# maxsonate/video-diffusion-nnx

Measured on AMD Instinct MI355X. Metric: denoised frames/sec, 16fx64x64 1000-step DDPM, higher is better.
Workload: dtype bf16; 1 GPU; config_v2_2 (north-star shape): Unet3D dim=64 C=1, 16f x 64x64, DDPM T=1000 p_sample_loop (UNet forward + p_sample per step, hipGraph replay); value = n_gpus*B*F/(T*s_per_step); batch_per_gpu=64, parallelism=dp1 (independent samples, no collective), mfma_operands=bf16, storage=weights fp32 master, activations bf16, fp32 accumulate, process_group=none (single process)

## Files before the change

video_diffusion_nnx_amd/csrc/conv_igemm.hip:

```cpp
#include "vdx_common.h"
#include <type_traits>
#include "vdx_internal.h"
#include "vdx_glds.h"
#include "model.h"
#include <stdlib.h>
#include <string.h>

namespace vdx {

typedef unsigned u32x4 __attribute__((ext_vector_type(4)));
typedef unsigned u32x2 __attribute__((ext_vector_type(2)));
constexpr unsigned OOB = 0xFFFFFFF0u;

template <int MODE, int BC, int TN, int NW, int INF>
__global__ __launch_bounds__(64 * NW, (NW == 8 && TN == 2) ? 4 : 2) void conv_igemm_kernel(const ConvArgs P) {
    using M = Mma<MODE>;
    constexpr int KT = M::KT;
    constexpr int RS = ROW_STRIDE;
    constexpr int WAVES_C = BC / 64;
    constexpr int WAVES_P = NW / WAVES_C;
    constexpr int NT = 64 * NW;
    constexpr int TM = 4;
    constexpr int APIECES = KT / 4;
    constexpr int WREGS = BC * 8 / NT;
// ... 689 lines not shown
        }
        {
            const int oy0 = tyc * 16 + 2 * wave, ox = txc * 16 + lp;
#pragma unroll
            for (int tn = 0; tn < 2; ++tn) {
                const size_t gout = ((size_t)(fcur * P.H + oy0 + tn) * P.W + ox) * 64;
#pragma unroll
                for (int tm = 0; tm < 4; ++tm) {
                    float4 v = make_float4(acc[tm][tn][0] + bias4[tm].x, acc[tm][tn][1] + bias4[tm].y, acc[tm][tn][2] + bias4[tm].z, acc[tm][tn][3] + bias4[tm].w);
                    const float4 r4 = rpre[tm][tn]; v.x += r4.x; v.y += r4.y; v.z += r4.z; v.w += r4.w;
                    store4_f32_or_bf16(P.y, gout + tm * 16 + 4 * q, v, OUT16 ? 1 : 0);
                    ssum[tm][0] += v.x; ssum[tm][1] += v.y; ssum[tm][2] += v.z; ssum[tm][3] += v.w;
                    ssq[tm][0] += v.x * v.x; ssq[tm][1] += v.y * v.y; ssq[tm][2] += v.z * v.z; ssq[tm][3] += v.w * v.w;
                }
            }
        }
        wait_vm<8>();
        if (more && bn != bcur) { flush_stats(bcur); bcur = bn; }
        fcur = fn; tyc = tyn; txc = txn;
        __syncthreads();
    }
    flush_stats(bcur);
}

template <typename K>
static hipError_t launch_tiles16(K kfn, const ConvArgs& a, size_t lds, long slots, hipStream_t st) {
    const int total = a.NF * (a.H >> 4) * (a.W >> 4);
    const PersistentSplit s = persistent_split(total, slots);
    if (hipError_t e = lds_opt_in(kfn, lds); e != hipSuccess) return e;
    hipLaunchKernelGGL(kfn, dim3((unsigned)s.workers), dim3(512), lds, st, a, (int)s.per, total);
    return hipGetLastError();
}

static hipError_t launch_conv64d(const ConvArgs& a, hipStream_t st) {
    if (a.pro || !a.x0_bf16 || !a.res || a.res_bf16) return hipErrorInvalidValue;
    const size_t lds = 9 * 64 * 128 + 2 * (size_t)C64D_APL + 128 * 8;
    return launch_tiles16(a.y_bf16 ? conv64d_kernel<true, true> : conv64d_kernel<false, true>, a, lds, device_cus(), st);
}

template <bool OUT16>
__global__ __launch_bounds__(512) void conv64r_kernel(const ConvArgs P, const int tiles_per_block, const int total_tiles) {
    using M = Mma<MODE_BF16>;
    constexpr int NDMA = 41, NK = (NDMA + 7) / 8;
    extern __shared__ __attribute__((aligned(16))) char smem[];
    char* Al = smem;
    double* chs = reinterpret_cast<double*>(Al + 3 * C64D_APL);
    float* biasl = reinterpret_cast<float*>(chs + 128);

    const int tid = threadIdx.x, lane = tid & 63;
    const int wave_u = __builtin_amdgcn_readfirstlane(tid >> 6);
    const int wc = wave_u & 1, wp = wave_u >> 1;
    const int lp = lane & 15, q = lane >> 4;
    const int tiles_x = P.W >> 4, tiles_pf = tiles_x * (P.H >> 4);
    const int t0 = blockIdx.x * tiles_per_block, t1 = min(t0 + tiles_per_block, total_tiles);
    if (t0 >= t1) return;

    uint4 wf[9][2][2];
#pragma unroll
    for (int tap = 0; tap < 9; ++tap)
#pragma unroll
        for (int ch = 0; ch < 2; ++ch)
#pragma unroll
            for (int tm = 0; tm < 2; ++tm)
                wf[tap][ch][tm] = *reinterpret_cast<const uint4*>(reinterpret_cast<const char*>(P.wp) +
                    ((size_t)tap * P.wrows + P.wrow0 + wc * 32 + 8 * (lp >> 2) + 4 * tm + (lp & 3)) * 128 + ch * 64 + q * 16);
    if (tid < 128) chs[tid] = 0.0;
    if (tid < 64) biasl[tid] = P.bias ? P.bias[tid] : 0.f;

    const char* const zero_page = reinterpret_cast<const char*>(g_zero_page_c64d);
    const char* const xb = reinterpret_cast<const char*>(P.x0);
    const unsigned al_base = lds_addr(Al);
    auto decode = [&](int t, int& f, int& ty, int& tx) { f = t / tiles_pf; const int r = t - f * tiles_pf; ty = r / tiles_x; tx = r - ty * tiles_x; };
    auto dma = [&](int t, int buf) {
        int f, ty, tx; decode(t, f, ty, tx);
        int ln = lane;
        asm volatile("" : "+v"(ln));
        const unsigned dst = al_base + buf * C64D_APL + wave_u * 1024;
#pragma unroll
        for (int k = 0; k < NK; ++k) {
            if (wave_u + 8 * k >= NDMA) continue;
            const int hp = (wave_u + 8 * k) * 8 + (ln >> 3);
            const int hy = (hp * 3641) >> 16, hx = hp - hy * 18;
            const int gy = ty * 16 - 1 + hy, gx = tx * 16 - 1 + hx;
            const bool ok = hp < C64_HALO && gy >= 0 && gy < P.H && gx >= 0 && gx < P.W;
            const size_t off = (size_t)((f * P.H + gy) * P.W + gx) * 128 + (((ln & 7) ^ (hx & 7)) << 4);
            glds16(ok ? static_cast<const void*>(xb + off) : static_cast<const void*>(zero_page), dst + k * 8 * 1024);
        }
    };
    const __amdgpu_buffer_rsrc_t rsy = __builtin_amdgcn_make_buffer_rsrc(P.y, 0, (unsigned)P.NF * P.H * P.W * 64u * (OUT16 ? 2u : 4u), 0x00020000);
    f32x4 ssum[2], ssq[2];
#pragma unroll
    for (int i = 0; i < 2; ++i) { ssum[i] = f32x4{0.f, 0.f, 0.f, 0.f}; ssq[i] = f32x4{0.f, 0.f, 0.f, 0.f}; }
    auto flush_stats = [&](int b) {
        if (!P.out_stats) return;
#pragma unroll
        for (int tm = 0; tm < 2; ++tm)
#pragma unroll
            for (int e = 0; e < 4; ++e) {
                const float s1 = reduce16(ssum[tm][e]), s2 = reduce16(ssq[tm][e]);
                const int c = wc * 32 + 8 * q + 4 * tm + e;
                if (lp == 0) { unsafeAtomicAdd(&chs[c], (double)s1); unsafeAtomicAdd(&chs[64 + c], (double)s2); }
                ssum[tm][e] = 0.f; ssq[tm][e] = 0.f;
            }
        __syncthreads();
        const int cpg = 64 / P.out_groups;
        int tt = tid;
        asm volatile("" : "+v"(tt));
        if (tt < 2 * P.out_groups) {
            const int g = tt >> 1, which = tt & 1;
            double t = 0.0;
            for (int c = g * cpg; c < (g + 1) * cpg; ++c) t += chs[which * 64 + c];
            unsafeAtomicAdd(P.out_stats + (((size_t)b * GN_SLOTS + (blockIdx.x % GN_SLOTS)) * P.out_groups + g) * 2 + which, t);
        }
        __syncthreads();
        if (tid < 128) chs[tid] = 0.0;
        __syncthreads();
    };

    int bdx[3][2];
#pragma unroll
    for (int ch = 0; ch < 2; ++ch)
#pragma unroll
        for (int dx = 0; dx < 3; ++dx) { const int hx = lp + dx; bdx[dx][ch] = hx * 128 + 16 * ((q + 4 * ch) ^ (hx & 7)); }
    const int rowbase = (4 * wp) * 18 * 128;

    int fcur, tyc, txc;
    decode(t0, fcur, tyc, txc);
    int bcur = fcur / P.F;
    __syncthreads();
    dma(t0, 0);
    if (t0 + 1 < t1) { dma(t0 + 1, 1); wait_vm<5>(); } else wait_vm<0>();
    __syncthreads();
    int buf = 0;
    for (int t = t0; t < t1; ++t) {
        const bool more = t + 1 < t1, more2 = t + 2 < t1;
        int fn = fcur, tyn = tyc, txn = txc, bn = bcur;
        if (more) { decode(t + 1, fn, tyn, txn); bn = fn / P.F; }
        if (more2) dma(t + 2, buf >= 1 ? buf - 1 : 2);
        const char* At = Al + buf * C64D_APL + rowbase;
        const int oy0 = tyc * 16 + 4 * wp, ox = txc * 16 + lp;
        f32x4 acc[2][4];
        uint4 bf[2][3];
        auto frag_read = [&](uint4 (&d)[3], int hr, int ch) {
#pragma unroll
            for (int dx = 0; dx < 3; ++dx) d[dx] = *reinterpret_cast<const uint4*>(At + bdx[dx][ch] + hr * (18 * 128));
        };
        frag_read(bf[0], 0, 0);
#pragma unroll
        for (int hr = 0; hr < 6; ++hr) {
            if (hr < 4) { acc[0][hr] = f32x4{0.f, 0.f, 0.f, 0.f}; acc[1][hr] = f32x4{0.f, 0.f, 0.f, 0.f}; }
#pragma unroll
            for (int ch = 0; ch < 2; ++ch) {
                const int s_ = 2 * hr + ch;
                if (s_ + 1 < 12) frag_read(bf[(s_ + 1) & 1], (s_ + 1) >> 1, (s_ + 1) & 1);
                __builtin_amdgcn_sched_barrier(0);
#pragma unroll
                for (int dx = 0; dx < 3; ++dx)
#pragma unroll
                    for (int dy = 0; dy < 3; ++dy) {
                        const int tn = hr - dy;
                        if (tn < 0 || tn > 3) continue;
#pragma unroll
                        for (int tm = 0; tm < 2; ++tm) M::mma(acc[tm][tn], wf[dy * 3 + dx][ch][tm], bf[s_ & 1][dx]);
                    }
                __builtin_amdgcn_sched_barrier(0);
            }
            if (hr >= 2) {
                const int tn = hr - 2;
                float4 bias4[2];
#pragma unroll
                for (int tm = 0; tm < 2; ++tm) bias4[tm] = *reinterpret_cast<const float4*>(biasl + wc * 32 + 8 * q + 4 * tm);
                const unsigned gout = (unsigned)(((fcur * P.H + oy0 + tn) * P.W + ox) * 64 + wc * 32 + 8 * q);
                float4 v[2];
#pragma unroll
                for (int tm = 0; tm < 2; ++tm) {
                    v[tm] = make_float4(acc[tm][tn][0] + bias4[tm].x, acc[tm][tn][1] + bias4[tm].y, acc[tm][tn][2] + bias4[tm].z, acc[tm][tn][3] + bias4[tm].w);
                    ssum[tm][0] += v[tm].x; ssum[tm][1] += v[tm].y; ssum[tm][2] += v[tm].z; ssum[tm][3] += v[tm].w;
                    ssq[tm][0] += v[tm].x * v[tm].x; ssq[tm][1] += v[tm].y * v[tm].y; ssq[tm][2] += v[tm].z * v[tm].z; ssq[tm][3] += v[tm].w * v[tm].w;
                }
                if constexpr (OUT16)
                    __builtin_amdgcn_raw_buffer_store_b128(u32x4{pack_bf16x2(v[0].x, v[0].y), pack_bf16x2(v[0].z, v[0].w), pack_bf16x2(v[1].x, v[1].y), pack_bf16x2(v[1].z, v[1].w)}, rsy, gout * 2u, 0, 0);
                else {
#pragma unroll
                    for (int tm = 0; tm < 2; ++tm)
                        __builtin_amdgcn_raw_buffer_store_b128(u32x4{__float_as_uint(v[tm].x), __float_as_uint(v[tm].y), __float_as_uint(v[tm].z), __float_as_uint(v[tm].w)}, rsy, (gout + 4 * tm) * 4u, 0, 0);
                }
            }
        }
        constexpr int NST = OUT16 ? 4 : 8;
        if (more2) wait_vm<5 + NST>(); else wait_vm<NST>();
        if (more && bn != bcur) { flush_stats(bcur); bcur = bn; }
        fcur = fn; tyc = tyn; txc = txn;
        buf = buf == 2 ? 0 : buf + 1;
        __syncthreads();
    }
    flush_stats(bcur);
}

static hipError_t launch_conv64r(const ConvArgs& a, hipStream_t st) {
    if (a.pro || !a.x0_bf16 || a.res) return hipErrorInvalidValue;
    const size_t lds = 3 * (size_t)C64D_APL + 128 * 8 + 64 * 4;
    return launch_tiles16(a.y_bf16 ? conv64r_kernel<true> : conv64r_kernel<false>, a, lds, device_cus(), st);
}

#ifndef VDX_C64Q_VPM
#define VDX_C64Q_VPM 6
#endif
template <int CIN, bool PRO, bool OUT16, int COUT = 64>
__global__ __launch_bounds__(512) void conv64q_kernel(const ConvArgs P, const int tiles_per_block, const int total_tiles) {
    using M = Mma<MODE_BF16>;
    static_assert(CIN == 64 || (CIN == 128 && !PRO), "prologue form: 64 input channels");
    static_assert(COUT == 64 || (COUT == 32 && !PRO), "COUT");
    constexpr int NWC = COUT / 16, NWP = 8 / NWC, RW = 16 / NWP, NHR = RW + 2, NSTEP = 2 * NHR;
    constexpr int NPL = CIN / 64;
    constexpr int NDMA = 41, NK = (NDMA + 7) / 8;
    constexpr int NST = (OUT16 ? 1 : 2) * (RW / 2);
    extern __shared__ __attribute__((aligned(16))) char smem[];
    char* Al = smem;
    double* chs = reinterpret_cast<double*>(Al + 3 * C64D_APL);
    float* biasl = reinterpret_cast<float*>(chs + 128);
    float* coefA = biasl + 64;
    float* coefD = coefA + 64;
    float* gmean = coefD + 64;

    const int tid = threadIdx.x, lane = tid & 63;
    const int wave_u = __builtin_amdgcn_readfirstlane(tid >> 6);
    const int wc = wave_u % NWC, wp = wave_u / NWC;
    const int lp = lane & 15, q = lane >> 4;
    const int tiles_x = P.W >> 4, tiles_pf = tiles_x * (P.H >> 4);
    const int t0 = blockIdx.x * tiles_per_block, t1 = min(t0 + tiles_per_block, total_tiles);
    if (t0 >= t1) return;

    uint4 wf[9][CIN / 32];
#pragma unroll
    for (int tap = 0; tap < 9; ++tap)
#pragma unroll
        for (int c = 0; c < CIN / 32; ++c)
            wf[tap][c] = *reinterpret_cast<const uint4*>(reinterpret_cast<const char*>(P.wp) +
                ((size_t)tap * P.wrows + P.wrow0 + wc * 16 + lp) * (CIN * 2) + c * 64 + q * 16);
    if (tid < 128) chs[tid] = 0.0;
    if (tid < 64) biasl[tid] = (P.bias && tid < COUT) ? P.bias[tid] : 0.f;

    const char* const zero_page = reinterpret_cast<const char*>(g_zero_page_c64d);
    const char* const xb0 = reinterpret_cast<const char*>(P.x0);
    const char* const xb1 = (CIN == 128) ? (P.C1 ? reinterpret_cast<const char*>(P.x1) : xb0 + 128) : xb0;
    const int rowb = (CIN == 128 && !P.C1) ? 256 : 128;
    const bool split32 = CIN == 64 && P.C1 == 32;
    const char* const xs1 = split32 ? reinterpret_cast<const char*>(P.x1) : nullptr;
    const unsigned al_base = lds_addr(Al);
    auto decode = [&](int t, int& f, int& ty, int& tx) { f = t / tiles_pf; const int r = t - f * tiles_pf; ty = r / tiles_x; tx = r - ty * tiles_x; };
    auto dma = [&](int t, int plane, int buf) {
        int f, ty, tx; decode(t, f, ty, tx);
        int ln = lane;
        asm volatile("" : "+v"(ln));
        const char* const xb = plane ? xb1 : xb0;
        const unsigned dst = al_base + buf * C64D_APL + wave_u * 1024;
#pragma unroll
        for (int k = 0; k < NK; ++k) {
            if (wave_u + 8 * k >= NDMA) continue;
            const int hp = (wave_u + 8 * k) * 8 + (ln >> 3);
            const int hy = (hp * 3641) >> 16, hx = hp - hy * 18;
            const int gy = ty * 16 - 1 + hy, gx = tx * 16 - 1 + hx;
            const bool ok = hp < C64_HALO && gy >= 0 && gy < P.H && gx >= 0 && gx < P.W;
            const int cch = (ln & 7) ^ (hx & 7);
            const size_t pixi = (size_t)((f * P.H + gy) * P.W + gx);
            const char* src = split32 ? (cch < 4 ? xb0 : xs1) + pixi * 64 + ((cch & 3) << 4) : xb + pixi * rowb + (cch << 4);
            glds16(ok ? static_cast<const void*>(src) : static_cast<const void*>(zero_page), dst + k * 8 * 1024);
        }
    };
    const __amdgpu_buffer_rsrc_t rsy = __builtin_amdgcn_make_buffer_rsrc(P.y, 0, (unsigned)P.NF * P.H * P.W * (unsigned)COUT * (OUT16 ? 2u : 4u), 0x00020000);
    float ssum[8], ssq[8];
#pragma unroll
    for (int i = 0; i < 8; ++i) { ssum[i] = 0.f; ssq[i] = 0.f; }
    auto flush_stats = [&](int b) {
        if (!P.out_stats) return;
#pragma unroll
        for (int i = 0; i < 8; ++i) {
            const float s1 = reduce16(ssum[i]), s2 = reduce16(ssq[i]);
            const int c = wc * 16 + 8 * (q >> 1) + i;
            if (lp == 0) { unsafeAtomicAdd(&chs[c], (double)s1); unsafeAtomicAdd(&chs[64 + c], (double)s2); }
            ssum[i] = 0.f; ssq[i] = 0.f;
        }
        __syncthreads();
        const int cpg = COUT / P.out_groups;
        int tt = tid;
        asm volatile("" : "+v"(tt));
        if (tt < 2 * P.out_groups) {
            const int g = tt >> 1, which = tt & 1;
            double t = 0.0;
            for (int c = g * cpg; c < (g + 1) * cpg; ++c) t += chs[which * 64 + c];
            unsafeAtomicAdd(P.out_stats + (((size_t)b * GN_SLOTS + (blockIdx.x % GN_SLOTS)) * P.out_groups + g) * 2 + which, t);
        }
        __syncthreads();
        if (tid < 128) chs[tid] = 0.0;
        __syncthreads();
    };
    const int tch = tid & 7, trow = tid >> 3;
    float ca[PRO ? 8 : 1], cd[PRO ? 8 : 1];
    auto make_coef = [&](int b) {
        if constexpr (PRO) {
            gn_mean_rstd_wg(P.in_stats, b, P.groups, (double)P.F * P.H * P.W * (64 / P.groups), gmean, tid, 512);
            __syncthreads();
            int tt = tid;
            asm volatile("" : "+v"(tt));
            if (tt < 64) {
                const int g = tt / (64 / P.groups);
                const float m = gmean[2 * g], rsd = gmean[2 * g + 1];
                float sc = 1.f, sh = 0.f;
                if (P.ss) { sc = P.ss[(size_t)b * P.ss_stride + tt] + 1.f; sh = P.ss[(size_t)b * P.ss_stride + 64 + tt]; }
                coefA[tt] = rsd * P.gamma[tt] * sc;
                coefD[tt] = (P.beta[tt] - m * rsd * P.gamma[tt]) * sc + sh;
            }
            __syncthreads();
#pragma unroll
            for (int i = 0; i < 8; ++i) { ca[i] = coefA[8 * tch + i]; cd[i] = coefD[8 * tch + i]; }
        }
    };
    auto piece_off = [&](int k) __attribute__((always_inline)) -> int {
        const int hp = trow + 64 * k;
        const int hy = (hp * 3641) >> 16, hx = hp - hy * 18;
        return hp * 128 + ((tch ^ (hx & 7)) << 4);
    };
    auto piece_ok = [&](int k, int ty, int tx) __attribute__((always_inline)) -> bool {
        const int hp = trow + 64 * k;
// ... 101 lines not shown
                                if ((c & 1) == 0) {
                                    cur = pv; okc = pok;
                                    if (k + 1 < NPK - 1) { pv = *reinterpret_cast<const u32x4*>(An + piece_off(k + 1)); pok = piece_ok(k + 1, tyn, txn); }
                                    half_math(cur.x, cur.y, 0, okc, oh0, oh1);
                                } else {
                                    unsigned o2, o3;
                                    half_math(cur.z, cur.w, 4, okc, o2, o3);
                                    *reinterpret_cast<u32x4*>(An + piece_off(k)) = u32x4{oh0, oh1, o2, o3};
                                }
#pragma unroll
                                for (int i = 0; i < 9; ++i) { __builtin_amdgcn_sched_group_barrier(0x008, 1, 0); __builtin_amdgcn_sched_group_barrier(0x002, VDX_C64Q_VPM, 0); }
                            }
                        }
                        __builtin_amdgcn_sched_barrier(0);
                        if constexpr (XF) {
                            if (s_ == 14 && wave_u == 0 && trow + 64 * (NPK - 1) < C64D_AROWS) {
                                char* pp = An + piece_off(NPK - 1);
                                *reinterpret_cast<u32x4*>(pp) = piece_math(*reinterpret_cast<const u32x4*>(pp), piece_ok(NPK - 1, tyn, txn));
                            }
                        }
                    }
                    if (plane == NPL - 1 && hr >= 3 && (hr & 1)) {
                        const int ta = hr - 3;
                        float v[8];
#pragma unroll
                        for (int r = 0; r < 4; ++r) {
                            const auto sw = __builtin_amdgcn_permlane16_swap(__float_as_uint(acc[ta][r]), __float_as_uint(acc[ta + 1][r]), false, false);
                            v[r] = __uint_as_float(sw[0]); v[4 + r] = __uint_as_float(sw[1]);
                        }
                        const float4 b0 = *reinterpret_cast<const float4*>(biasl + wc * 16 + 8 * (q >> 1)), b1 = *reinterpret_cast<const float4*>(biasl + wc * 16 + 8 * (q >> 1) + 4);
                        v[0] += b0.x; v[1] += b0.y; v[2] += b0.z; v[3] += b0.w; v[4] += b1.x; v[5] += b1.y; v[6] += b1.z; v[7] += b1.w;
#pragma unroll
                        for (int i = 0; i < 8; ++i) { ssum[i] += v[i]; ssq[i] += v[i] * v[i]; }
                        const unsigned gout = (unsigned)(((fcur * P.H + oy0 + ta + (q & 1)) * P.W + ox) * COUT + wc * 16 + 8 * (q >> 1));
                        if constexpr (OUT16)
                            __builtin_amdgcn_raw_buffer_store_b128(u32x4{pack_bf16x2(v[0], v[1]), pack_bf16x2(v[2], v[3]), pack_bf16x2(v[4], v[5]), pack_bf16x2(v[6], v[7])}, rsy, gout * 2u, 0, 0);
                        else {
                            __builtin_amdgcn_raw_buffer_store_b128(u32x4{__float_as_uint(v[0]), __float_as_uint(v[1]), __float_as_uint(v[2]), __float_as_uint(v[3])}, rsy, gout * 4u, 0, 0);
                            __builtin_amdgcn_raw_buffer_store_b128(u32x4{__float_as_uint(v[4]), __float_as_uint(v[5]), __float_as_uint(v[6]), __float_as_uint(v[7])}, rsy, (gout + 4) * 4u, 0, 0);
                        }
                    }
                }
            };
            if (PRO && more) steps(std::true_type{}); else steps(std::false_type{});
            if constexpr (PRO) wait_vm<NST>();
            else {
                const bool issued = j + 2 < npass;
                if (plane == NPL - 1) { if (issued) wait_vm<5 + NST>(); else wait_vm<NST>(); }
                else { if (issued) wait_vm<5>(); else wait_vm<0>(); }
            }
            if (plane == NPL - 1) {
                if (more && bn != bcur) { flush_stats(bcur); bcur = bn; }
                if constexpr (PRO) {
                    if (t + 2 < t1) { int f2, ty2, tx2; decode(t + 2, f2, ty2, tx2); const int b2 = f2 / P.F; if (b2 != bcoef) { make_coef(b2); bcoef = b2; } }
                }
            }
            buf = bufn;
            __syncthreads();
        }
        fcur = fn; tyc = tyn; txc = txn;
    }
    flush_stats(bcur);
}

static hipError_t launch_conv64q(const ConvArgs& a, hipStream_t st) {
    if (!a.x0_bf16 || a.res || (a.C1 && !a.x1_bf16)) return hipErrorInvalidValue;
    const size_t lds = 3 * (size_t)C64D_APL + 128 * 8 + 64 * 4 + (64 + 64 + 64) * 4;
    auto launch = [&](auto kfn) { return launch_tiles16(kfn, a, lds, device_cus(), st); };
    if (a.Cout == 32) {
        if (a.pro || !a.y_bf16) return hipErrorInvalidValue;
        return a.C0 + a.C1 == 128 ? launch(conv64q_kernel<128, false, true, 32>) : launch(conv64q_kernel<64, false, true, 32>);
    }
    if (a.C0 + a.C1 == 128) {
        if (a.pro) return hipErrorInvalidValue;
        return a.y_bf16 ? launch(conv64q_kernel<128, false, true>) : launch(conv64q_kernel<128, false, false>);
    }
    if (!a.pro) return hipErrorInvalidValue;
    return a.y_bf16 ? launch(conv64q_kernel<64, true, true>) : launch(conv64q_kernel<64, true, false>);
}

static hipError_t launch_conv64p(const ConvArgs& a, hipStream_t st) {
    if (a.res) return hipErrorInvalidValue;
    if (a.Cout == 32) {
        if (!a.x0_bf16 || !a.y_bf16) return hipErrorInvalidValue;
        const size_t lds = 9 * 32 * 64 + 2 * (size_t)C64_HALO * 64 + (64 + 64 + 64) * 4 + 128 * 8 + 64 * 4;
        const long slots = (long)((a.pro ? VDX_C32_PRO_WAVES : 4) / 2) * device_cus();
        return launch_tiles16(a.pro ? conv64p_kernel<true, true, true, false, 32> : conv64p_kernel<true, false, true, false, 32>, a, lds, slots, st);
    }
    if (a.x0_bf16) return hipErrorInvalidValue;
    const size_t lds = 9 * 64 * 128 + 2 * (size_t)C64_HALO * 128 + (64 + 64 + 64) * 4 + 128 * 8 + 64 * 4;
    auto launch = [&](auto kfn) { return launch_tiles16(kfn, a, lds, device_cus(), st); };
    if (a.pro) return a.y_bf16 ? launch(conv64p_kernel<false, true, true>) : launch(conv64p_kernel<false, true, false>);
    return a.y_bf16 ? launch(conv64p_kernel<false, false, true>) : launch(conv64p_kernel<false, false, false>);
}

template <int MODE>
__global__ void pack_weights_kernel(const float* __restrict__ src, void* __restrict__ dst, int taps, int Cin, int Cout, int CinPad) {
    const size_t n = (size_t)taps * Cout * CinPad;
    for (size_t i = (size_t)blockIdx.x * blockDim.x + threadIdx.x; i < n; i += (size_t)gridDim.x * blockDim.x) {
        const int ci = (int)(i % CinPad);
        const size_t r = i / CinPad;
        const int co = (int)(r % Cout);
        const int t = (int)(r / Cout);
        const float v = (ci < Cin) ? src[((size_t)t * Cin + ci) * Cout + co] : 0.f;
        store_operand<MODE>(dst, i, v);
    }
}
// ... 140 lines not shown
             a.NF, a.H, a.W, a.stride == 2 ? " s2" : "", a.pro ? " +prologue" : "", a.res ? " +res" : "", a.C1 ? " concat" : "");
    return w;
}
}

static bool tiles16_3x3(int mode, const ConvArgs& a) {
    return mode == MODE_BF16 && a.kind == 0 && a.kh == 3 && a.kw == 3 && a.stride == 1 && a.H % 16 == 0 && a.W % 16 == 0 &&
           (long)a.NF * (a.H / 16) * (a.W / 16) >= 1024;
}
static bool conv64_shape(int mode, const ConvArgs& a) {
    return tiles16_3x3(mode, a) && a.C0 == 64 && a.C1 == 0 && a.Cout == 64 && a.wrows >= 64 && a.wrow0 >= 0 && a.wrow0 + 64 <= a.wrows &&
           (!a.res || (!a.pro && a.x0_bf16 && !a.res_bf16)) && (size_t)a.NF * a.H * a.W * 64 * (a.y_bf16 ? 2 : 4) < 0xFFFFFFF0ull &&
           (!a.pro || (a.groups <= 32 && 64 % a.groups == 0)) && (!a.out_stats || (a.out_groups <= 32 && 64 % a.out_groups == 0));
}
static bool conv64q_pro_eligible(int mode, const ConvArgs& a) { return conv64_shape(mode, a) && a.x0_bf16 && a.pro; }
static bool conv64r_eligible(int mode, const ConvArgs& a) { return conv64_shape(mode, a) && a.x0_bf16 && !a.pro && !a.res; }
static bool conv64d_eligible(int mode, const ConvArgs& a) { return conv64_shape(mode, a) && a.x0_bf16 && !a.pro && a.res; }
static bool conv64p_eligible(int mode, const ConvArgs& a) { return conv64_shape(mode, a) && !a.x0_bf16; }
static bool conv64p_c32_eligible(int mode, const ConvArgs& a) {
    return tiles16_3x3(mode, a) && a.C0 == 32 && a.C1 == 0 && a.Cout == 32 && a.wrows == 32 && a.wrow0 == 0 && a.CinPad == 64 && a.x0_bf16 &&
           a.y_bf16 && !a.res && (!a.pro || (a.groups <= 32 && 32 % a.groups == 0)) && (!a.out_stats || (a.out_groups <= 32 && 32 % a.out_groups == 0));
}
static bool conv64q_cout32_eligible(int mode, const ConvArgs& a) {
    return tiles16_3x3(mode, a) && a.Cout == 32 && a.x0_bf16 && a.x1_bf16 && !a.pro && a.y_bf16 && ((a.C0 == 32 && a.C1 == 32) || (a.C0 == 64 && a.C1 == 64)) &&
           a.CinPad == a.C0 + a.C1 && a.wrows == 32 && a.wrow0 == 0 && !a.res &&
           (!a.out_stats || (a.out_groups <= 32 && 32 % a.out_groups == 0 && (32 / a.out_groups) <= 8 && 8 % (32 / a.out_groups) == 0));
}
static bool conv64q_cin128_eligible(int mode, const ConvArgs& a) {
    return tiles16_3x3(mode, a) && a.Cout == 64 && a.x0_bf16 && (!a.C1 || a.x1_bf16) && !a.pro && ((a.C0 == 64 && a.C1 == 64) || (a.C0 == 128 && a.C1 == 0)) &&
           a.wrows == 64 && a.wrow0 == 0 && !a.res && (!a.out_stats || (a.out_groups <= 32 && 32 % (64 / a.out_groups) == 0 && 64 % a.out_groups == 0)) &&
           (long)a.NF * a.H * a.W * 256 < 0xFFFFFFF0l;
}

hipError_t launch_conv(int mode, ConvArgs a, hipStream_t st) {
    const int K = a.kind ? 2 : a.kh;
    if (a.kind) { a.stride = 1; a.Ho = a.H; a.Wo = a.W; a.Hy = 2 * a.H; a.Wy = 2 * a.W; }
    else { a.Ho = (a.H + a.stride - 1) / a.stride; a.Wo = (a.W + a.stride - 1) / a.stride; a.Hy = a.Ho; a.Wy = a.Wo; }
    a.CinPad = conv_cin_pad(mode, a.C0 + a.C1);
    const int ES = mode == MODE_F32 ? 4 : 2;
    const size_t npix = (size_t)a.NF * a.H * a.W;
    if (a.wrows <= 0) { a.wrows = a.Cout; a.wrow0 = 0; }
    const size_t b0 = npix * a.C0 * (a.x0_bf16 ? 2 : 4), b1 = npix * a.C1 * (a.x1_bf16 ? 2 : 4), bw = (size_t)(a.kind ? 16 : a.kh * a.kw) * a.wrows * a.CinPad * ES;
    if (b0 >= 0xFFFFFFF0ull || b1 >= 0xFFFFFFF0ull || bw >= 0xFFFFFFF0ull) return hipErrorInvalidValue;
    a.x0_bytes = (unsigned)b0; a.x1_bytes = (unsigned)b1; a.w_bytes = (unsigned)bw;
    if (conv3x3_ws_eligible(mode, a)) {
        const ConvWork cw = conv_work(mode, a);
        LaunchScope ls(st, "conv3x3_ws_kernel", cw.flops, cw.bytes, "<%d, %s> %s", conv3x3_ws_geo(a), a.pro ? "true" : "false", cw.shape);
        return launch_conv3x3_ws(a, st);
    }
    if (conv4x4_ws_eligible(mode, a)) {
        const ConvWork cw = conv_work(mode, a);
        LaunchScope ls(st, "conv4x4_ws_kernel", cw.flops, cw.bytes, "<%d, %d, %d> %s", a.kind == 1 ? a.H : a.H / 2, a.kind == 1 ? 2 : 1, a.Cout == 64 ? 64 : 128, cw.shape);
        return launch_conv4x4_ws(a, st);
    }
    if (resample32_eligible(mode, a)) {
        const ConvWork cw = conv_work(mode, a);
        LaunchScope ls(st, "resample32_kernel", cw.flops, cw.bytes, "<%d> %s", a.kind, cw.shape);
        return launch_resample32(a, st);
    }
    if (conv1x1_pw_eligible(mode, a)) {
        const ConvWork cw = conv_work(mode, a);
        LaunchScope ls(st, "conv1x1_pw_kernel", cw.flops, cw.bytes, "<%d> %s", conv1x1_pw_rows(a), cw.shape);
        return launch_conv1x1_pw(a, st);
    }
    if (conv64q_pro_eligible(mode, a)) {
        const ConvWork cw = conv_work(mode, a);
        LaunchScope ls(st, "conv64q_kernel", cw.flops, cw.bytes, "<cin 64, pro %d, y16 %d> %s", a.pro, a.y_bf16, cw.shape);
        return launch_conv64q(a, st);
    }
    if (conv64r_eligible(mode, a)) {
        const ConvWork cw = conv_work(mode, a);
        LaunchScope ls(st, "conv64r_kernel", cw.flops, cw.bytes, "<pro 0, y16 %d> %s", a.y_bf16, cw.shape);
        return launch_conv64r(a, st);
    }
    if (conv64d_eligible(mode, a)) {
        const ConvWork cw = conv_work(mode, a);
        LaunchScope ls(st, "conv64d_kernel", cw.flops, cw.bytes, "<x16 %d, pro %d, y16 %d, res %d> %s", a.x0_bf16, a.pro, a.y_bf16, a.res ? 1 : 0, cw.shape);
// ... 69 lines not shown
```

video_diffusion_nnx_amd/csrc/model.hip:

```cpp
#include <math.h>
#include <stdio.h>
#include <string.h>
#include <string>
#include <vector>

#include "vdx_common.h"
#include "vdx_internal.h"
#include "model.h"
#include <stdlib.h>

namespace vdx {

static long add_param(Model* m, const std::string& name, std::initializer_list<long> shape) {
    ParamInfo p;
    p.name = name;
    p.ndim = (int)shape.size();
    long n = 1;
    int i = 0;
    for (long s : shape) { p.shape[i++] = s; n *= s; }
    p.offset = m->param_total;
    p.numel = n;
    m->param_total += (n + 3) / 4 * 4;
    m->params.push_back(p);
    return p.offset;
// ... 307 lines not shown
    float* act; float* temb; float* ss; float* ss_lin; double* stats; char* sla_ws;
    float* slot(int s) const { return act + (size_t)m->slots[s].offset_per_sample * B; }
    double* stat(int i) const { return stats + (size_t)i * B * GN_SLOTS * m->cfg.resnet_groups * 2; }
};

#ifndef VDX_PREPASS_MIN_C
#define VDX_PREPASS_MIN_C 256
#endif

static hipError_t run_res(const Fwd& f, const ResP& r, const float* x0, int c0, const float* x1, int c1, int lvl, float* head_out = nullptr, bool* head_done = nullptr) {
    const Model* m = f.m;
    const int G = m->cfg.resnet_groups;
    const int S = m->cfg.image_size >> lvl;
    ConvArgs a;
    memset(&a, 0, sizeof(a));
    a.x0 = x0; a.x1 = x1; a.C0 = c0; a.C1 = c1;
    a.wp = f.pk + r.pk_b1; a.bias = f.p + r.b1_b; a.y = f.slot(r.s_y1); a.Cout = r.cout;
    a.NF = f.B * m->cfg.num_frames; a.F = m->cfg.num_frames; a.H = S; a.W = S;
    a.kind = 0; a.kh = a.kw = 3; a.stride = 1; a.pad = 1;
    a.out_stats = f.stat(r.st1); a.out_groups = G;
    const int half = (m->mode == MODE_BF16);
    a.y_bf16 = half; a.x0_bf16 = f.a16; a.x1_bf16 = f.a16;
    hipError_t e = launch_conv(m->mode, a, f.st);
    if (e != hipSuccess) return e;
    ConvArgs b;
    memset(&b, 0, sizeof(b));
    b.x0 = f.slot(r.s_y1); b.C0 = r.cout;
    b.wp = f.pk + r.pk_b2; b.bias = f.p + r.b2_b; b.y = f.slot(r.s_y2); b.Cout = r.cout;
    b.NF = a.NF; b.F = a.F; b.H = S; b.W = S; b.kind = 0; b.kh = b.kw = 3; b.stride = 1; b.pad = 1;
    b.x0_bf16 = half; b.y_bf16 = half;
    b.pro = 1; b.in_stats = f.stat(r.st1); b.gamma = f.p + r.b1_gs; b.beta = f.p + r.b1_gb; b.groups = G;
    if (r.has_mlp) { b.ss = f.ss + (size_t)m->ss_layers[r.ss_index].out_off * f.B; b.ss_stride = 2 * r.cout; }
    b.out_stats = f.stat(r.st2); b.out_groups = G;
    if (half && m->act16 == 1 && r.cout >= VDX_PREPASS_MIN_C) {
        e = launch_gn_silu_apply16(f.slot(r.s_y1), b.in_stats, b.gamma, b.beta, b.ss, b.ss_stride, G, r.cout, f.B, (long)m->cfg.num_frames * S * S, f.st);
        if (e != hipSuccess) return e;
        b.pro = 0; b.in_stats = nullptr; b.gamma = b.beta = nullptr; b.ss = nullptr; b.groups = 0;
    }
    e = launch_conv(m->mode, b, f.st);
    if (e != hipSuccess) return e;
    const float* rsrc = x0;
    const bool fuse_rc = r.has_res && f.a16 && m->act16 == 1 && m->mode == MODE_BF16 &&
                         tail_rc16_supported(c0 + c1, c0, r.cout, (long)m->cfg.num_frames * S * S);
    if (r.has_res && !fuse_rc) {
        ConvArgs c;
        memset(&c, 0, sizeof(c));
        c.x0 = x0; c.x1 = x1; c.C0 = c0; c.C1 = c1;
        c.wp = f.pk + r.pk_rc; c.bias = f.p + r.rc_b; c.y = f.slot(r.s_rc); c.Cout = r.cout;
        c.NF = a.NF; c.F = a.F; c.H = S; c.W = S; c.kind = 0; c.kh = c.kw = 1; c.stride = 1; c.pad = 0;
        c.x0_bf16 = f.a16; c.x1_bf16 = f.a16; c.y_bf16 = f.a16;
        e = launch_conv(m->mode, c, f.st);
        if (e != hipSuccess) return e;
        rsrc = f.slot(r.s_rc);
    }
    TailArgs t;
    memset(&t, 0, sizeof(t));
    t.y2 = f.slot(r.s_y2); t.y2_bf16 = half; t.r = rsrc; t.out = f.slot(r.s_out); t.r_bf16 = f.a16; t.out_bf16 = f.a16;
    t.stats = f.stat(r.st2); t.gn_gamma = f.p + r.b2_gs; t.gn_beta = f.p + r.b2_gb; t.groups = G;
    t.ln_gamma = f.p + r.n2_s; t.ln_beta = f.p + r.n2_b;
    t.C = r.cout; t.batch = f.B; t.pix_per_sample = (long)m->cfg.num_frames * S * S;
    if (fuse_rc) { t.x0 = x0; t.x1 = x1; t.C0 = c0; t.C1 = c1; t.rc_w = f.pk + r.pk_rc; t.rc_b = f.p + r.rc_b; }
    if (head_out && fuse_rc && c1 == c0 && m->out_dim == 1 && ((c0 + c1 == 128 && r.cout == 64) || (c0 + c1 == 64 && r.cout == 32))) {
        t.fin_w = f.p + m->fin_w; t.fin_b = f.p + m->fin_b; t.fin_out = head_out;
        *head_done = true;
    }
    return launch_resblock_tail(t, f.st);
}
// ... 177 lines not shown
```

video_diffusion_nnx_amd/csrc/vdx_internal.h:

```cpp
#pragma once
#include <hip/hip_runtime.h>
#include <stdarg.h>
#include <stddef.h>
#include <stdio.h>
#include <algorithm>
#include "../../include/vdx.h"

int vdx_set_error(int code, const char* msg, const char* file, int line);

namespace vdx {

extern vdx_launch_hook g_launch_hook;
extern void* g_launch_hook_user;
struct LaunchScope {
    vdx_launch_info info; char desc[192]; hipStream_t st; bool on;
    LaunchScope(hipStream_t s, const char* kernel, double flops, double bytes, const char* fmt, ...) __attribute__((format(printf, 6, 7))) : st(s), on(g_launch_hook != nullptr) {
        if (!on) return;
        va_list ap;
        va_start(ap, fmt);
        vsnprintf(desc, sizeof(desc), fmt, ap);
        va_end(ap);
        info.kernel = kernel; info.shape = desc; info.flops = flops; info.bytes = bytes;
        g_launch_hook(g_launch_hook_user, 0, &info, st);
    }
// ... 12 lines not shown
inline PersistentSplit persistent_split(long total, long slots) {
    const long n = std::min(total, slots);
    const long per = (total + n - 1) / n;
    return {per, (total + per - 1) / per};
}

template <typename K>
inline hipError_t lds_opt_in(K kfn, size_t lds) {
    if (lds <= 64 * 1024) return hipSuccess;
    return hipFuncSetAttribute(reinterpret_cast<const void*>(kfn), hipFuncAttributeMaxDynamicSharedMemorySize, (int)lds);
}

struct ConvArgs {
    const float* x0; const float* x1; int C0, C1;
    const void* wp;
    const float* bias;
    float* y; int Cout;
    int NF, F;
    int H, W;
    int kind;
    int kh, kw, stride, pad;
    int pro;
    const double* in_stats; const float* gamma; const float* beta; int groups;
    const float* ss; int ss_stride;
    double* out_stats; int out_groups;
    int x0_bf16, y_bf16;
    int x1_bf16;
    const float* res;
    int res_bf16;
    int wrows, wrow0;
    int Ho, Wo, Hy, Wy, CinPad, PH, PW, NP, tiles_y, tiles_x;
    unsigned x0_bytes, x1_bytes, w_bytes;
    unsigned m_ihiw, m_iw, m_phpw, m_pw;
};

struct TailArgs {
    const float* y2; const float* r; float* out;
    int y2_bf16;
    int r_bf16, out_bf16;
    const double* stats; const float* gn_gamma; const float* gn_beta; int groups;
    const float* ln_gamma; const float* ln_beta;
    int C; int batch; long pix_per_sample;
    int lpp;
    const float* x0; const float* x1; int C0, C1;
    const void* rc_w;
    const float* rc_b;
    const float* fin_w; const float* fin_b; float* fin_out;
};
bool tail_rc16_supported(int cin, int c0, int cout, long pix_per_sample);

struct TimeMlpArgs {
    const int* time; int t_is_device_scalar;
    const float* w1; const float* b1; const float* w2; const float* b2;
    int dim, time_dim;
    const float* cond; const float* null_cond_emb; const unsigned char* cond_mask; int null_all; int cond_dim;
    float* temb; int temb_dim;
};

struct SsLayer { long w_off, b_off, g_off, be_off, out_off; int n; int pad_; };

hipError_t launch_resblock_tail(TailArgs a, hipStream_t st);
hipError_t launch_init_conv(const float* x, const float* w, const float* bias, float* y, int B, int Cin, int F, int H, int W,
                            int Cout, int K, int y_bf16, hipStream_t st);
hipError_t launch_init_conv_mode(int mode, const float* x, const float* w, const float* bias, float* y, int B, int Cin, int F, int H, int W,
                                 int Cout, int K, int y_bf16, hipStream_t st);
hipError_t launch_final_conv(const float* x, const float* w, const float* bias, float* y, long npix, int D, int Cout, int x_bf16, hipStream_t st);
// ... 154 lines not shown
size_t attn_bwd_bias_scratch_floats(int heads, int L);
hipError_t launch_attn_core_bwd(const AttnBwdArgs& a, hipStream_t st);
hipError_t launch_pos_bias_scatter(const float* dbias, const int* buckets, float* demb, int heads, int n, hipStream_t st);
struct AttnBwdXArgs {
    const float* x; const float* g;
    int x_bf16;
    const void* wqkv; const float* bqkv;
    const void* woT;
    void* O; void* dqkv;
    float* dx;
    int L; long nseq, inner, outer_p, tok_p; float scale;
};
hipError_t launch_attn_bwd_fused(const AttnBwdXArgs& a, hipStream_t st);
struct SlaBwdArgs {
    const float* q; const float* k; const float* v; const float* dOut; float* O; float* dq; float* dk; float* dv; float* A;
    int NF, N, heads;
    int dstride;
    int io_bf16;
    int bf16_mma;
};
size_t sla_bwd_scratch_floats(int NF, int heads);
hipError_t launch_sla_bwd(const SlaBwdArgs& a, hipStream_t st);

hipError_t launch_final_conv_bwd(const float* x, const float* dout, const float* w, float* dx, float* dW, float* db, long npix, int D, int Cout, int x_bf16, hipStream_t st, float* part = nullptr, size_t part_cap = 0);
hipError_t launch_init_conv_wgrad(const float* x, const float* dy, float* dW, float* db, int B, int Cin, int F, int H, int W, int Cout, int K, hipStream_t st, float* part = nullptr, size_t part_cap = 0);
hipError_t launch_resblock_ss_bwd(const float* params, float* grads, const float* temb, const SsLayer* layers, int nlayers, const float* lin_base,
                                  float* dss_base, float* dtemb, int temb_dim, int B, hipStream_t st, float* part = nullptr, size_t part_cap = 0);
hipError_t launch_time_mlp_bwd(const TimeMlpArgs& a, const float* dtemb, float* dw1, float* db1, float* dw2, float* db2, float* dnull, int B, hipStream_t st);

size_t conv_packed_bytes(int mode, int taps, int Cin, int Cout);
int conv_cin_pad(int mode, int Cin);
hipError_t launch_pack_weights(int mode, const float* src, void* dst, int taps, int Cin, int Cout, hipStream_t st);
hipError_t launch_conv(int mode, ConvArgs a, hipStream_t st);
int conv3x3_ws_geo(const ConvArgs& a);
bool conv4x4_ws_eligible(int mode, const ConvArgs& a);
hipError_t launch_conv4x4_ws(const ConvArgs& a, hipStream_t st);
hipError_t launch_gn_silu_apply16(float* y_bf16, const double* stats, const float* gamma, const float* beta, const float* ss, int ss_stride, int groups,
                                  int C, int batch, long pix_per_sample, hipStream_t st);
bool resample32_eligible(int mode, const ConvArgs& a);
hipError_t launch_resample32(const ConvArgs& a, hipStream_t st);
bool conv1x1_pw_eligible(int mode, const ConvArgs& a);
hipError_t launch_conv1x1_pw(const ConvArgs& a, hipStream_t st);
int conv1x1_pw_rows(const ConvArgs& a);
bool conv3x3_ws_eligible(int mode, const ConvArgs& a);
hipError_t launch_conv3x3_ws(const ConvArgs& a, hipStream_t st);
hipError_t launch_pack_weights_t(int mode, const float* src, void* dst, int taps, int Cin, int Cout, hipStream_t st);

}
```

video_diffusion_nnx_amd/ops.py:

```python
from __future__ import annotations

import ctypes as C

import torch

from . import _lib as L


def _mode(mode) -> int:
    return L.MODES[mode] if isinstance(mode, str) else int(mode)


def _is16(t) -> int:
    assert t.dtype in (torch.float32, torch.bfloat16)
    return int(t.dtype == torch.bfloat16)


def pack_conv_weights(kernel: torch.Tensor, mode) -> torch.Tensor:
    m = _mode(mode)
    cin, cout = kernel.shape[-2], kernel.shape[-1]
    taps = kernel.numel() // (cin * cout)
    k = kernel.contiguous().float()
    n = L.vdx_packed_conv_bytes(m, taps, cin, cout)
    out = torch.empty(n, dtype=torch.uint8, device=k.device)
    L.check(L.vdx_pack_conv_weights(m, L.ptr(k), L.ptr(out), taps, cin, cout, L.stream_ptr()))
    return out


def gn_stats_zeros(batch: int, groups: int, device) -> torch.Tensor:
    return torch.zeros(batch * L.GN_SLOTS * groups * 2, dtype=torch.float64, device=device)


def gn_stats_reduce(stats: torch.Tensor, batch: int, groups: int) -> torch.Tensor:
    return stats.view(batch, L.GN_SLOTS, groups, 2).sum(1)


def conv_forward(x0, packed_w, cout, *, mode, bias=None, x1=None, kind=0, k=3, stride=1,
                 in_stats=None, gamma=None, beta=None, groups=8, scale_shift=None,
                 out_stats=None, out_groups=8, y_bf16=False, res=None) -> torch.Tensor:
    B, Fr, H, W, c0 = x0.shape
    c1 = 0 if x1 is None else x1.shape[-1]
    if kind == 1:
        Ho, Wo = 2 * H, 2 * W
    else:
        Ho, Wo = -(-H // stride), -(-W // stride)
    x_bf16 = x0.dtype == torch.bfloat16
    assert x0.dtype in (torch.float32, torch.bfloat16) and (x1 is None or x1.dtype == x0.dtype)
    y = torch.empty(B, Fr, Ho, Wo, cout, dtype=torch.bfloat16 if y_bf16 else torch.float32, device=x0.device)
    d = L.ConvDesc()
    d.x_bf16, d.y_bf16 = int(x_bf16), int(bool(y_bf16))
    d.x0, d.x1, d.c0, d.c1 = L.ptr(x0), L.ptr(x1), c0, c1
    d.packed_w, d.bias, d.y, d.cout = L.ptr(packed_w), L.ptr(bias), L.ptr(y), cout
    d.batch, d.frames, d.h, d.w = B, Fr, H, W
    d.kind, d.kh, d.kw, d.stride = kind, k, k, stride
    d.in_stats, d.gamma, d.beta, d.groups = L.ptr(in_stats), L.ptr(gamma), L.ptr(beta), groups
    d.scale_shift = L.ptr(scale_shift)
    d.scale_shift_stride = 0 if scale_shift is None else scale_shift.shape[-1]
    d.out_stats, d.out_groups = L.ptr(out_stats), out_groups
    d.res, d.res_bf16 = L.ptr(res), int(res is not None and res.dtype == torch.bfloat16)
    L.check(L.vdx_conv_forward(_mode(mode), C.byref(d), L.stream_ptr()))
    return y


def resblock_tail(y2, r, stats, gn_gamma, gn_beta, ln_gamma, ln_beta, groups=8):
    B, C = y2.shape[0], y2.shape[-1]
    pix = y2.numel() // (B * C)
    out = torch.empty_like(y2)
    L.check(L.vdx_resblock_tail(L.ptr(y2), L.ptr(r), L.ptr(out), L.ptr(stats), L.ptr(gn_gamma), L.ptr(gn_beta), groups,
                                L.ptr(ln_gamma), L.ptr(ln_beta), C, B, pix, L.stream_ptr()))
    return out


def _pack_rc(rc_kernel):
    cin = rc_kernel.shape[0]
    wp = rc_kernel.t().contiguous().to(torch.bfloat16)
    if cin % 64:
        wp = torch.nn.functional.pad(wp, (0, 64 - cin % 64)).contiguous()
    return wp


def resblock_tail_rc_bf16(y2, x0, x1, rc_kernel, rc_bias, stats, gn_gamma, gn_beta, ln_gamma, ln_beta, groups=8):
# ... 546 lines not shown
```

Baseline: 49.91 frames/s.

## Route 128/256-out-channel 3x3 convs to 64-channel kernels via output-channel slicing

Adds a sliced launch mode where the specialized conv64r/conv64q kernels each compute one 64-channel slice of a wider output (Cout 128 or 256). Slices are interleaved with XCD-aware block mapping, and GroupNorm stats are written per slice. For 128-channel resblocks, a GN+SiLU prepass is now forced so the no-prologue sliced kernel can be used. The aim is to replace the generic path for these shapes with the faster hand-tuned kernels. The cost is that the input tile is reloaded once per slice, plus the extra prepass traffic.

```diff
diff --git a/video_diffusion_nnx_amd/csrc/conv_igemm.hip b/video_diffusion_nnx_amd/csrc/conv_igemm.hip
--- a/video_diffusion_nnx_amd/csrc/conv_igemm.hip
+++ b/video_diffusion_nnx_amd/csrc/conv_igemm.hip
@@ -745,13 +745,31 @@
     return hipGetLastError();
 }
 
+struct SliceId { int slice, range; };
+template <bool SL>
+__device__ __forceinline__ SliceId slice_id(const ConvArgs& P) {
+    if constexpr (!SL) return {0, (int)blockIdx.x};
+    else { const int xcd = blockIdx.x & 7, slot = blockIdx.x >> 3; return {slot % P.nslice, (slot / P.nslice) * 8 + xcd}; }
+}
+template <typename K>
+static hipError_t launch_tiles16_slices(K kfn, const ConvArgs& a, size_t lds, hipStream_t st) {
+    const int total = a.NF * (a.H >> 4) * (a.W >> 4);
+    const int unit = 8 * a.nslice;
+    const long nranges = std::max(unit, device_cus() / unit * unit) / a.nslice;
+    const PersistentSplit s = persistent_split(total, nranges);
+    if (hipError_t e = lds_opt_in(kfn, lds); e != hipSuccess) return e;
+    const unsigned grid = (unsigned)((s.workers + 7) / 8 * 8 * a.nslice);
+    hipLaunchKernelGGL(kfn, dim3(grid), dim3(512), lds, st, a, (int)s.per, total);
+    return hipGetLastError();
+}
+
 static hipError_t launch_conv64d(const ConvArgs& a, hipStream_t st) {
     if (a.pro || !a.x0_bf16 || !a.res || a.res_bf16) return hipErrorInvalidValue;
     const size_t lds = 9 * 64 * 128 + 2 * (size_t)C64D_APL + 128 * 8;
     return launch_tiles16(a.y_bf16 ? conv64d_kernel<true, true> : conv64d_kernel<false, true>, a, lds, device_cus(), st);
 }
 
-template <bool OUT16>
+template <bool OUT16, bool SL = false>
 __global__ __launch_bounds__(512) void conv64r_kernel(const ConvArgs P, const int tiles_per_block, const int total_tiles) {
     using M = Mma<MODE_BF16>;
     constexpr int NDMA = 41, NK = (NDMA + 7) / 8;
@@ -765,7 +783,9 @@
     const int wc = wave_u & 1, wp = wave_u >> 1;
     const int lp = lane & 15, q = lane >> 4;
     const int tiles_x = P.W >> 4, tiles_pf = tiles_x * (P.H >> 4);
-    const int t0 = blockIdx.x * tiles_per_block, t1 = min(t0 + tiles_per_block, total_tiles);
+    const SliceId sid = slice_id<SL>(P);
+    const int ch0 = 64 * sid.slice, ys = SL ? P.ystride : 64;
+    const int t0 = sid.range * tiles_per_block, t1 = min(t0 + tiles_per_block, total_tiles);
     if (t0 >= t1) return;
 
     uint4 wf[9][2][2];
@@ -776,9 +796,9 @@
 #pragma unroll
             for (int tm = 0; tm < 2; ++tm)
                 wf[tap][ch][tm] = *reinterpret_cast<const uint4*>(reinterpret_cast<const char*>(P.wp) +
-                    ((size_t)tap * P.wrows + P.wrow0 + wc * 32 + 8 * (lp >> 2) + 4 * tm + (lp & 3)) * 128 + ch * 64 + q * 16);
+                    ((size_t)tap * P.wrows + P.wrow0 + ch0 + wc * 32 + 8 * (lp >> 2) + 4 * tm + (lp & 3)) * 128 + ch * 64 + q * 16);
     if (tid < 128) chs[tid] = 0.0;
-    if (tid < 64) biasl[tid] = P.bias ? P.bias[tid] : 0.f;
+    if (tid < 64) biasl[tid] = P.bias ? P.bias[ch0 + tid] : 0.f;
 
     const char* const zero_page = reinterpret_cast<const char*>(g_zero_page_c64d);
     const char* const xb = reinterpret_cast<const char*>(P.x0);
@@ -800,7 +820,7 @@
             glds16(ok ? static_cast<const void*>(xb + off) : static_cast<const void*>(zero_page), dst + k * 8 * 1024);
         }
     };
-    const __amdgpu_buffer_rsrc_t rsy = __builtin_amdgcn_make_buffer_rsrc(P.y, 0, (unsigned)P.NF * P.H * P.W * 64u * (OUT16 ? 2u : 4u), 0x00020000);
+    const __amdgpu_buffer_rsrc_t rsy = __builtin_amdgcn_make_buffer_rsrc(P.y, 0, (unsigned)P.NF * P.H * P.W * (unsigned)ys * (OUT16 ? 2u : 4u), 0x00020000);
     f32x4 ssum[2], ssq[2];
 #pragma unroll
     for (int i = 0; i < 2; ++i) { ssum[i] = f32x4{0.f, 0.f, 0.f, 0.f}; ssq[i] = f32x4{0.f, 0.f, 0.f, 0.f}; }
@@ -816,14 +836,14 @@
                 ssum[tm][e] = 0.f; ssq[tm][e] = 0.f;
             }
         __syncthreads();
-        const int cpg = 64 / P.out_groups;
+        const int cpg = ys / P.out_groups, ngl = SL ? 64 / cpg : P.out_groups;
         int tt = tid;
         asm volatile("" : "+v"(tt));
-        if (tt < 2 * P.out_groups) {
+        if (tt < 2 * ngl) {
             const int g = tt >> 1, which = tt & 1;
             double t = 0.0;
             for (int c = g * cpg; c < (g + 1) * cpg; ++c) t += chs[which * 64 + c];
-            unsafeAtomicAdd(P.out_stats + (((size_t)b * GN_SLOTS + (blockIdx.x % GN_SLOTS)) * P.out_groups + g) * 2 + which, t);
+            unsafeAtomicAdd(P.out_stats + (((size_t)b * GN_SLOTS + (blockIdx.x % GN_SLOTS)) * P.out_groups + sid.slice * ngl + g) * 2 + which, t);
         }
         __syncthreads();
         if (tid < 128) chs[tid] = 0.0;
@@ -883,7 +903,7 @@
                 float4 bias4[2];
 #pragma unroll
                 for (int tm = 0; tm < 2; ++tm) bias4[tm] = *reinterpret_cast<const float4*>(biasl + wc * 32 + 8 * q + 4 * tm);
-                const unsigned gout = (unsigned)(((fcur * P.H + oy0 + tn) * P.W + ox) * 64 + wc * 32 + 8 * q);
+                const unsigned gout = (unsigned)(((fcur * P.H + oy0 + tn) * P.W + ox) * ys + ch0 + wc * 32 + 8 * q);
                 float4 v[2];
 #pragma unroll
                 for (int tm = 0; tm < 2; ++tm) {
@@ -913,17 +933,19 @@
 static hipError_t launch_conv64r(const ConvArgs& a, hipStream_t st) {
     if (a.pro || !a.x0_bf16 || a.res) return hipErrorInvalidValue;
     const size_t lds = 3 * (size_t)C64D_APL + 128 * 8 + 64 * 4;
+    if (a.nslice > 1) return a.y_bf16 ? launch_tiles16_slices(conv64r_kernel<true, true>, a, lds, st) : hipErrorInvalidValue;
     return launch_tiles16(a.y_bf16 ? conv64r_kernel<true> : conv64r_kernel<false>, a, lds, device_cus(), st);
 }
 
 #ifndef VDX_C64Q_VPM
 #define VDX_C64Q_VPM 6
 #endif
-template <int CIN, bool PRO, bool OUT16, int COUT = 64>
+template <int CIN, bool PRO, bool OUT16, int COUT = 64, bool SL = false>
 __global__ __launch_bounds__(512) void conv64q_kernel(const ConvArgs P, const int tiles_per_block, const int total_tiles) {
     using M = Mma<MODE_BF16>;
     static_assert(CIN == 64 || (CIN == 128 && !PRO), "prologue form: 64 input channels");
     static_assert(COUT == 64 || (COUT == 32 && !PRO), "COUT");
+    static_assert(!SL || (CIN == 128 && COUT == 64 && !PRO), "sliced form");
     constexpr int NWC = COUT / 16, NWP = 8 / NWC, RW = 16 / NWP, NHR = RW + 2, NSTEP = 2 * NHR;
     constexpr int NPL = CIN / 64;
     constexpr int NDMA = 41, NK = (NDMA + 7) / 8;
@@ -941,7 +963,9 @@
     const int wc = wave_u % NWC, wp = wave_u / NWC;
     const int lp = lane & 15, q = lane >> 4;
     const int tiles_x = P.W >> 4, tiles_pf = tiles_x * (P.H >> 4);
-    const int t0 = blockIdx.x * tiles_per_block, t1 = min(t0 + tiles_per_block, total_tiles);
+    const SliceId sid = slice_id<SL>(P);
+    const int ch0 = 64 * sid.slice, ys = SL ? P.ystride : COUT;
+    const int t0 = sid.range * tiles_per_block, t1 = min(t0 + tiles_per_block, total_tiles);
     if (t0 >= t1) return;
 
     uint4 wf[9][CIN / 32];
@@ -950,9 +974,9 @@
 #pragma unroll
         for (int c = 0; c < CIN / 32; ++c)
             wf[tap][c] = *reinterpret_cast<const uint4*>(reinterpret_cast<const char*>(P.wp) +
-                ((size_t)tap * P.wrows + P.wrow0 + wc * 16 + lp) * (CIN * 2) + c * 64 + q * 16);
+                ((size_t)tap * P.wrows + P.wrow0 + ch0 + wc * 16 + lp) * (CIN * 2) + c * 64 + q * 16);
     if (tid < 128) chs[tid] = 0.0;
-    if (tid < 64) biasl[tid] = (P.bias && tid < COUT) ? P.bias[tid] : 0.f;
+    if (tid < 64) biasl[tid] = (P.bias && tid < COUT) ? P.bias[ch0 + tid] : 0.f;
 
     const char* const zero_page = reinterpret_cast<const char*>(g_zero_page_c64d);
     const char* const xb0 = reinterpret_cast<const char*>(P.x0);
@@ -981,7 +1005,7 @@
             glds16(ok ? static_cast<const void*>(src) : static_cast<const void*>(zero_page), dst + k * 8 * 1024);
         }
     };
-    const __amdgpu_buffer_rsrc_t rsy = __builtin_amdgcn_make_buffer_rsrc(P.y, 0, (unsigned)P.NF * P.H * P.W * (unsigned)COUT * (OUT16 ? 2u : 4u), 0x00020000);
+    const __amdgpu_buffer_rsrc_t rsy = __builtin_amdgcn_make_buffer_rsrc(P.y, 0, (unsigned)P.NF * P.H * P.W * (unsigned)ys * (OUT16 ? 2u : 4u), 0x00020000);
     float ssum[8], ssq[8];
 #pragma unroll
     for (int i = 0; i < 8; ++i) { ssum[i] = 0.f; ssq[i] = 0.f; }
@@ -995,14 +1019,14 @@
             ssum[i] = 0.f; ssq[i] = 0.f;
         }
         __syncthreads();
-        const int cpg = COUT / P.out_groups;
+        const int cpg = ys / P.out_groups, ngl = SL ? 64 / cpg : P.out_groups;
         int tt = tid;
         asm volatile("" : "+v"(tt));
-        if (tt < 2 * P.out_groups) {
+        if (tt < 2 * ngl) {
             const int g = tt >> 1, which = tt & 1;
             double t = 0.0;
             for (int c = g * cpg; c < (g + 1) * cpg; ++c) t += chs[which * 64 + c];
-            unsafeAtomicAdd(P.out_stats + (((size_t)b * GN_SLOTS + (blockIdx.x % GN_SLOTS)) * P.out_groups + g) * 2 + which, t);
+            unsafeAtomicAdd(P.out_stats + (((size_t)b * GN_SLOTS + (blockIdx.x % GN_SLOTS)) * P.out_groups + sid.slice * ngl + g) * 2 + which, t);
         }
         __syncthreads();
         if (tid < 128) chs[tid] = 0.0;
@@ -1170,7 +1194,7 @@
                         v[0] += b0.x; v[1] += b0.y; v[2] += b0.z; v[3] += b0.w; v[4] += b1.x; v[5] += b1.y; v[6] += b1.z; v[7] += b1.w;
 #pragma unroll
                         for (int i = 0; i < 8; ++i) { ssum[i] += v[i]; ssq[i] += v[i] * v[i]; }
-                        const unsigned gout = (unsigned)(((fcur * P.H + oy0 + ta + (q & 1)) * P.W + ox) * COUT + wc * 16 + 8 * (q >> 1));
+                        const unsigned gout = (unsigned)(((fcur * P.H + oy0 + ta + (q & 1)) * P.W + ox) * ys + ch0 + wc * 16 + 8 * (q >> 1));
                         if constexpr (OUT16)
                             __builtin_amdgcn_raw_buffer_store_b128(u32x4{pack_bf16x2(v[0], v[1]), pack_bf16x2(v[2], v[3]), pack_bf16x2(v[4], v[5]), pack_bf16x2(v[6], v[7])}, rsy, gout * 2u, 0, 0);
                         else {
@@ -1211,6 +1235,7 @@
     }
     if (a.C0 + a.C1 == 128) {
         if (a.pro) return hipErrorInvalidValue;
+        if (a.nslice > 1) return a.y_bf16 ? launch_tiles16_slices(conv64q_kernel<128, false, true, 64, true>, a, lds, st) : hipErrorInvalidValue;
         return a.y_bf16 ? launch(conv64q_kernel<128, false, true>) : launch(conv64q_kernel<128, false, false>);
     }
     if (!a.pro) return hipErrorInvalidValue;
@@ -1417,6 +1442,21 @@
            (long)a.NF * a.H * a.W * 256 < 0xFFFFFFF0l;
 }
 
+bool conv64_slices_shape(int mode, int cin, int cout, int NF, int H, int W, int out_groups) {
+    if (mode != MODE_BF16 || (cin != 64 && cin != 128) || (cout != 128 && cout != 256) || H % 16 || W % 16) return false;
+    if ((long)NF * (H / 16) * (W / 16) < 1024) return false;
+    if (out_groups) {
+        if (out_groups < 1 || cout % out_groups) return false;
+        const int cpg = cout / out_groups;
+        if (cpg > 64 || 64 % cpg) return false;
+    }
+    return (long)NF * H * W * 256 < 0xFFFFFFF0l && (size_t)NF * H * W * cout * 2 < 0xFFFFFFF0ull;
+}
+static bool conv64_slices_eligible(int mode, const ConvArgs& a) {
+    return tiles16_3x3(mode, a) && a.x0_bf16 && a.y_bf16 && !a.pro && !a.res && a.C1 == 0 && a.CinPad == a.C0 && a.wrows == a.Cout && a.wrow0 == 0 &&
+           (!a.out_stats || a.out_groups >= 1) && conv64_slices_shape(mode, a.C0, a.Cout, a.NF, a.H, a.W, a.out_stats ? a.out_groups : 0);
+}
+
 hipError_t launch_conv(int mode, ConvArgs a, hipStream_t st) {
     const int K = a.kind ? 2 : a.kh;
     if (a.kind) { a.stride = 1; a.Ho = a.H; a.Wo = a.W; a.Hy = 2 * a.H; a.Wy = 2 * a.W; }
@@ -1428,6 +1468,17 @@
     const size_t b0 = npix * a.C0 * (a.x0_bf16 ? 2 : 4), b1 = npix * a.C1 * (a.x1_bf16 ? 2 : 4), bw = (size_t)(a.kind ? 16 : a.kh * a.kw) * a.wrows * a.CinPad * ES;
     if (b0 >= 0xFFFFFFF0ull || b1 >= 0xFFFFFFF0ull || bw >= 0xFFFFFFF0ull) return hipErrorInvalidValue;
     a.x0_bytes = (unsigned)b0; a.x1_bytes = (unsigned)b1; a.w_bytes = (unsigned)bw;
+    a.ystride = a.Cout; a.nslice = 1;
+    if (conv64_slices_eligible(mode, a)) {
+        a.nslice = a.Cout / 64;
+        const ConvWork cw = conv_work(mode, a);
+        if (a.C0 == 64) {
+            LaunchScope ls(st, "conv64r_kernel", cw.flops, cw.bytes, "<pro 0, y16 1, slices %d> %s", a.nslice, cw.shape);
+            return launch_conv64r(a, st);
+        }
+        LaunchScope ls(st, "conv64q_kernel", cw.flops, cw.bytes, "<cin 128, pro 0, y16 1, slices %d> %s", a.nslice, cw.shape);
+        return launch_conv64q(a, st);
+    }
     if (conv3x3_ws_eligible(mode, a)) {
         const ConvWork cw = conv_work(mode, a);
         LaunchScope ls(st, "conv3x3_ws_kernel", cw.flops, cw.bytes, "<%d, %s> %s", conv3x3_ws_geo(a), a.pro ? "true" : "false", cw.shape);
diff --git a/video_diffusion_nnx_amd/csrc/model.hip b/video_diffusion_nnx_amd/csrc/model.hip
--- a/video_diffusion_nnx_amd/csrc/model.hip
+++ b/video_diffusion_nnx_amd/csrc/model.hip
@@ -363,7 +363,8 @@
     b.pro = 1; b.in_stats = f.stat(r.st1); b.gamma = f.p + r.b1_gs; b.beta = f.p + r.b1_gb; b.groups = G;
     if (r.has_mlp) { b.ss = f.ss + (size_t)m->ss_layers[r.ss_index].out_off * f.B; b.ss_stride = 2 * r.cout; }
     b.out_stats = f.stat(r.st2); b.out_groups = G;
-    if (half && m->act16 == 1 && r.cout >= VDX_PREPASS_MIN_C) {
+    const bool pre128 = r.cout == 128 && conv64_slices_shape(m->mode, 128, 128, b.NF, S, S, G);
+    if (half && m->act16 == 1 && (r.cout >= VDX_PREPASS_MIN_C || pre128)) {
         e = launch_gn_silu_apply16(f.slot(r.s_y1), b.in_stats, b.gamma, b.beta, b.ss, b.ss_stride, G, r.cout, f.B, (long)m->cfg.num_frames * S * S, f.st);
         if (e != hipSuccess) return e;
         b.pro = 0; b.in_stats = nullptr; b.gamma = b.beta = nullptr; b.ss = nullptr; b.groups = 0;
diff --git a/video_diffusion_nnx_amd/csrc/vdx_internal.h b/video_diffusion_nnx_amd/csrc/vdx_internal.h
--- a/video_diffusion_nnx_amd/csrc/vdx_internal.h
+++ b/video_diffusion_nnx_amd/csrc/vdx_internal.h
@@ -68,6 +68,7 @@
     int Ho, Wo, Hy, Wy, CinPad, PH, PW, NP, tiles_y, tiles_x;
     unsigned x0_bytes, x1_bytes, w_bytes;
     unsigned m_ihiw, m_iw, m_phpw, m_pw;
+    int ystride, nslice;
 };
 
 struct TailArgs {
@@ -288,6 +289,7 @@
 int conv_cin_pad(int mode, int Cin);
 hipError_t launch_pack_weights(int mode, const float* src, void* dst, int taps, int Cin, int Cout, hipStream_t st);
 hipError_t launch_conv(int mode, ConvArgs a, hipStream_t st);
+bool conv64_slices_shape(int mode, int cin, int cout, int NF, int H, int W, int out_groups);
 int conv3x3_ws_geo(const ConvArgs& a);
 bool conv4x4_ws_eligible(int mode, const ConvArgs& a);
 hipError_t launch_conv4x4_ws(const ConvArgs& a, hipStream_t st);
diff --git a/video_diffusion_nnx_amd/ops.py b/video_diffusion_nnx_amd/ops.py
--- a/video_diffusion_nnx_amd/ops.py
+++ b/video_diffusion_nnx_amd/ops.py
@@ -37,7 +37,7 @@
 
 def conv_forward(x0, packed_w, cout, *, mode, bias=None, x1=None, kind=0, k=3, stride=1,
                  in_stats=None, gamma=None, beta=None, groups=8, scale_shift=None,
-                 out_stats=None, out_groups=8, y_bf16=False, res=None) -> torch.Tensor:
+                 out_stats=None, out_groups=8, y_bf16=False, res=None, out=None) -> torch.Tensor:
     B, Fr, H, W, c0 = x0.shape
     c1 = 0 if x1 is None else x1.shape[-1]
     if kind == 1:
@@ -46,7 +46,12 @@
         Ho, Wo = -(-H // stride), -(-W // stride)
     x_bf16 = x0.dtype == torch.bfloat16
     assert x0.dtype in (torch.float32, torch.bfloat16) and (x1 is None or x1.dtype == x0.dtype)
-    y = torch.empty(B, Fr, Ho, Wo, cout, dtype=torch.bfloat16 if y_bf16 else torch.float32, device=x0.device)
+    y_dtype = torch.bfloat16 if y_bf16 else torch.float32
+    if out is None:
+        y = torch.empty(B, Fr, Ho, Wo, cout, dtype=y_dtype, device=x0.device)
+    else:
+        assert out.shape == (B, Fr, Ho, Wo, cout) and out.dtype == y_dtype and out.is_contiguous() and out.device == x0.device
+        y = out
     d = L.ConvDesc()
     d.x_bf16, d.y_bf16 = int(x_bf16), int(bool(y_bf16))
     d.x0, d.x1, d.c0, d.c1 = L.ptr(x0), L.ptr(x1), c0, c1
```

New measurement: 50.60 frames/s, median of 6. +1.4%, better.
